# caki35/UNet-Torch

Measured on AMD Instinct MI355X. Metric: images/sec training step, 4-level U-Net 1ch→2cls 512×512, at 1/2/4/8 MI355X, higher is better.
Workload: dtype f16

## Files before the change

unet-torch_amd/csrc/generic_kernels.hip:

```cpp
#include "kernels.h"

template <typename T, bool K8>
__global__ void pack_kn_kernel(const float* __restrict__ src, T* __restrict__ dst, int Tn, int K, int N,
                               long st, long sk, long sn, int flip_t, int Kpad, int Npad) {
    long total = (long)Tn * Kpad * Npad;
    for (long i = (long)blockIdx.x * blockDim.x + threadIdx.x; i < total; i += (long)gridDim.x * blockDim.x) {
        int n, k, t;
        if (K8) {
            int k8 = (int)(i & 7);
            long r = i >> 3;
            n = (int)(r % Npad); r /= Npad;
            int kb = (int)(r % (Kpad / 8));
            t = (int)(r / (Kpad / 8));
            k = kb * 8 + k8;
        } else {
            n = (int)(i % Npad);
            long r = i / Npad;
            k = (int)(r % Kpad);
            t = (int)(r / Kpad);
        }
        float v = 0.f;
        if (k < K && n < N) {
            int ts = flip_t ? (Tn - 1 - t) : t;
            v = src[ts * st + k * sk + n * sn];
// ... 523 lines not shown
            vs[i] = ws[((long)rc * 2 + 0) * C + c];
            vq[i] = ws[((long)rc * 2 + w1) * C + c];
        }
#pragma unroll
        for (int i = 0; i < 8; ++i) asm volatile("" : "+v"(vs[i]), "+v"(vq[i]));
#pragma unroll
        for (int i = 0; i < 8; ++i) { const bool ok = r0 + 256 * i < rows; vs[i] = ok ? vs[i] : 0.f; vq[i] = (ok && out1) ? vq[i] : 0.f; }
#pragma unroll
        for (int i = 0; i < 8; ++i) { s += (double)vs[i]; q += (double)vq[i]; }
    }
    sh[0][tid] = s;
    sh[1][tid] = q;
    __syncthreads();
    for (int o = 128; o > 0; o >>= 1) {
        if (tid < o) { sh[0][tid] += sh[0][tid + o]; sh[1][tid] += sh[1][tid + o]; }
        __syncthreads();
    }
    if (tid == 0) {
        out0[c] = (float)(sh[0][0] * (double)scale);
        if (out1) out1[c] = (float)(sh[1][0] * (double)scale);
    }
}

__global__ __launch_bounds__(256) void reduce_rows2_2d_kernel(const float* __restrict__ ws, int rows, int C,
                                                              float* __restrict__ out0, float* __restrict__ out1,
                                                              float scale, int region) {
    double tot = 0.0;
    if (!red2d_block(ws, rows, C, out1 != nullptr, region, tot)) return;
    const int lane = threadIdx.x & 63, c = blockIdx.x * 32 + (lane & 31);
    if (c < C) {
        if (lane < 32) out0[c] = (float)(tot * (double)scale);
        else if (out1) out1[c] = (float)(tot * (double)scale);
    }
}

__global__ __launch_bounds__(256) void reduce_rows2_wide_kernel(const float* __restrict__ ws, int rows, int C,
                                                                float* __restrict__ out0, float* __restrict__ out1, float scale) {
    const int c = blockIdx.x * 256 + threadIdx.x;
    if (c >= C) return;
    double s = 0.0, q = 0.0;
    for (int r = 0; r < rows; ++r) {
        s += (double)ws[((long)r * 2 + 0) * C + c];
        if (out1) q += (double)ws[((long)r * 2 + 1) * C + c];
    }
    out0[c] = (float)(s * (double)scale);
    if (out1) out1[c] = (float)(q * (double)scale);
}

void umi_launch_reduce_rows2(const float* ws, int rows, int C, float* out0, float* out1, float scale, hipStream_t s) {
    if (rows <= 64 && C >= 4096)
        hipLaunchKernelGGL(reduce_rows2_wide_kernel, dim3((C + 255) / 256), dim3(256), 0, s, ws, rows, C, out0, out1, scale);
    else if (red2d_ok(rows, C))
        hipLaunchKernelGGL(reduce_rows2_2d_kernel, dim3((C + 31) / 32, (rows + RED_RPS - 1) / RED_RPS), dim3(256), 0, s, ws,
                           rows, C, out0, out1, scale, red2d_region());
    else
        hipLaunchKernelGGL(reduce_rows2_kernel, dim3(C), dim3(256), 0, s, ws, rows, C, out0, out1, scale);
}

template <typename T>
__global__ void bn_bwd_apply_kernel(T* __restrict__ da, int ldda, const T* __restrict__ y, int ldy,
                                    const float4* __restrict__ tx, const float* __restrict__ rstd,
                                    const float* __restrict__ sum_dz, const float* __restrict__ sum_dzx, long M, int C) {
    const float invM = 1.f / (float)M;
    long total = M * C;
    for (long i = (long)blockIdx.x * blockDim.x + threadIdx.x; i < total; i += (long)gridDim.x * blockDim.x) {
        int c = (int)(i % C);
        long r = i / C;
        da[r * ldda + c] = umi_bn_dz<T>((float)y[r * ldy + c], (float)da[r * ldda + c], tx[c], rstd[c], sum_dz[c] * invM,
                                        sum_dzx[c] * invM);
    }
}

extern "C" size_t umi_bn_bwd_ws_bytes(long M, int C) {
    const int a = umi_cdiv(M, BNB_RPB), b = umi_cdiv(M, umi_bn_bwd_rpb_f16v(M));
    return (size_t)(a > b ? a : b) * 2 * (size_t)C * sizeof(float);
}

extern "C" int umi_bn_bwd_reduce(const void* da, int ldda, const void* y, int ldy, const void* tx, const float* rstd,
                                 float* sum_dz, float* sum_dzx, long M, int C, int dtype, void* ws, size_t ws_bytes,
                                 umi_stream_t stream) {
    if (!da || !y || !tx || !rstd || M <= 0 || C <= 0) return UMI_ERR_BADARG;
    if (ws_bytes < umi_bn_bwd_ws_bytes(M, C)) return UMI_ERR_WORKSPACE;
    int rows = umi_cdiv(M, BNB_RPB);
    hipStream_t s = (hipStream_t)stream;
    if (dtype == UMI_F16 && umi_bn_bwd_reduce1_f16v(da, ldda, y, ldy, tx, rstd, (float*)ws, M, C, s)) {
        UMI_LAUNCH_CHECK();
        rows = umi_cdiv(M, umi_bn_bwd_rpb_f16v(M));
        umi_launch_reduce_rows2((const float*)ws, rows, C, sum_dz, sum_dzx, 1.f, s);
        UMI_LAUNCH_CHECK();
        return UMI_OK;
    }
    if (dtype == UMI_F32) hipLaunchKernelGGL(bn_bwd_reduce1_kernel<float>, dim3(rows), dim3(256), 0, s, (const float*)da, ldda, (const float*)y, ldy, (const float4*)tx, rstd, (float*)ws, M, C);
    else if (dtype == UMI_F16) hipLaunchKernelGGL(bn_bwd_reduce1_kernel<half_t>, dim3(rows), dim3(256), 0, s, (const half_t*)da, ldda, (const half_t*)y, ldy, (const float4*)tx, rstd, (float*)ws, M, C);
    else return UMI_ERR_BADARG;
    UMI_LAUNCH_CHECK();
    umi_launch_reduce_rows2((const float*)ws, rows, C, sum_dz, sum_dzx, 1.f, s);
    UMI_LAUNCH_CHECK();
    return UMI_OK;
}

extern "C" int umi_bn_bwd_apply(void* da, int ldda, const void* y, int ldy, const void* tx, const float* rstd,
                                const float* sum_dz, const float* sum_dzx, long M, int C, int dtype,
                                umi_stream_t stream) {
    if (!da || !y || !tx || !rstd || M <= 0 || C <= 0) return UMI_ERR_BADARG;
    long total = M * C;
    int grid = (int)((total + 255) / 256);
    if (grid > 16384) grid = 16384;
    hipStream_t s = (hipStream_t)stream;
    if (dtype == UMI_F16 && umi_bn_bwd_apply_f16v(da, ldda, y, ldy, tx, rstd, sum_dz, sum_dzx, M, C, s)) {
        UMI_LAUNCH_CHECK();
        return UMI_OK;
    }
    if (dtype == UMI_F32) hipLaunchKernelGGL(bn_bwd_apply_kernel<float>, dim3(grid), dim3(256), 0, s, (float*)da, ldda, (const float*)y, ldy, (const float4*)tx, rstd, sum_dz, sum_dzx, M, C);
    else if (dtype == UMI_F16) hipLaunchKernelGGL(bn_bwd_apply_kernel<half_t>, dim3(grid), dim3(256), 0, s, (half_t*)da, ldda, (const half_t*)y, ldy, (const float4*)tx, rstd, sum_dz, sum_dzx, M, C);
    else return UMI_ERR_BADARG;
    UMI_LAUNCH_CHECK();
    return UMI_OK;
}

template <typename T>
__global__ __launch_bounds__(256) void colsum1_kernel(const T* __restrict__ x, int ldx, float* __restrict__ ws, long M,
                                                      int C, long rows_per_split, float* __restrict__ out, float scale) {
    __shared__ float red[4][64];
    const int cl = threadIdx.x & 63, rl = threadIdx.x >> 6;
    const int c = blockIdx.x * 64 + cl;
    const long r0 = (long)blockIdx.y * rows_per_split;
    long r1 = r0 + rows_per_split;
    if (r1 > M) r1 = M;
    float s = 0.f;
    if (c < C)
        for (long r = r0 + rl; r < r1; r += 4) s += (float)x[r * ldx + c];
    red[rl][cl] = s;
    __syncthreads();
    if (rl == 0 && c < C) {
        const float t = red[0][cl] + red[1][cl] + red[2][cl] + red[3][cl];
        if (gridDim.y == 1) out[c] = t * scale;
        else ws[((long)blockIdx.y * 2 + 0) * C + c] = t;
    }
}

__global__ void fold_cols_kernel(const float* __restrict__ tmp8, int C, float* __restrict__ out, float scale) {
    const int c = threadIdx.x;
    if (c < C) {
        float s = 0.f;
        for (int k = c; k < 8; k += C) s += tmp8[k];
        out[c] = s * scale;
    }
}

static void colsum_plan(long M, int C, int* splits, long* rps) {
    long ctiles = (C + 63) / 64;
    long want = (1024 + ctiles - 1) / ctiles;
    long maxs = (M + 31) / 32;
    if (want > maxs) want = maxs;
    if (want < 1) want = 1;
    *rps = (M + want - 1) / want;
    *splits = (int)((M + *rps - 1) / *rps);
}

extern "C" size_t umi_colsum_ws_bytes(long M, int C) {
    int splits; long rps;
    colsum_plan(M, C, &splits, &rps);
    const int vrows = umi_colsum_rows_f16v(M, C);
    size_t b = (size_t)(splits > vrows ? splits : vrows) * 2 * (size_t)C * sizeof(float);
    if (C < 8 && 8 % C == 0 && (M * C) % 8 == 0) {
        const size_t b8 = ((size_t)umi_colsum_rows_f16v(M * C / 8, 8) * 2 * 8 + 8) * sizeof(float);
        if (b8 > b) b = b8;
    }
    return b;
}

extern "C" int umi_colsum_group(int n, const void* const* xs, int ldx, float* const* outs, float out_scale, long M, int C,
                                int dtype, void* ws, size_t ws_bytes, umi_stream_t stream) {
    if (n <= 0 || !xs || !outs || M <= 0 || C <= 0 || !ws) return UMI_ERR_BADARG;
    for (int i = 0; i < n; ++i)
        if (!xs[i] || !outs[i]) return UMI_ERR_BADARG;
    if (ws_bytes < (size_t)(n < 16 ? n : 16) * umi_colsum_ws_bytes(M, C)) return UMI_ERR_WORKSPACE;
    if (dtype != UMI_F16 || !umi_colsum_group_f16v(n, xs, ldx, outs, out_scale, (float*)ws, M, C, (hipStream_t)stream))
        return UMI_ERR_UNSUPPORTED;
    UMI_LAUNCH_CHECK();
    return UMI_OK;
}

extern "C" int umi_colsum(const void* x, int ldx, float* out, float out_scale, long M, int C, int dtype, void* ws,
                          size_t ws_bytes, umi_stream_t stream) {
    if (!x || !out || M <= 0 || C <= 0) return UMI_ERR_BADARG;
    if (ws_bytes < umi_colsum_ws_bytes(M, C)) return UMI_ERR_WORKSPACE;
    int splits; long rps;
    colsum_plan(M, C, &splits, &rps);
    hipStream_t s = (hipStream_t)stream;
    if (dtype == UMI_F16 && umi_colsum_f16v(x, ldx, (float*)ws, M, C, s)) {
        UMI_LAUNCH_CHECK();
        umi_launch_reduce_rows2((const float*)ws, umi_colsum_rows_f16v(M, C), C, out, (float*)nullptr, out_scale, s);
        UMI_LAUNCH_CHECK();
        return UMI_OK;
    }
    if (dtype == UMI_F16 && C < 8 && 8 % C == 0 && ldx == C && (M * C) % 8 == 0 &&
        ws_bytes >= ((size_t)umi_colsum_rows_f16v(M * C / 8, 8) * 2 * 8 + 8) * sizeof(float)) {
        const long M8 = M * C / 8;
        float* tmp = (float*)ws + (size_t)umi_colsum_rows_f16v(M8, 8) * 2 * 8;
        if (umi_colsum_f16v(x, 8, (float*)ws, M8, 8, s)) {
            UMI_LAUNCH_CHECK();
            umi_launch_reduce_rows2((const float*)ws, umi_colsum_rows_f16v(M8, 8), 8, tmp, (float*)nullptr, 1.f, s);
            hipLaunchKernelGGL(fold_cols_kernel, dim3(1), dim3(64), 0, s, (const float*)tmp, C, out, out_scale);
            UMI_LAUNCH_CHECK();
            return UMI_OK;
        }
    }
    dim3 grid((C + 63) / 64, splits);
    if (dtype == UMI_F32) hipLaunchKernelGGL(colsum1_kernel<float>, grid, dim3(256), 0, s, (const float*)x, ldx, (float*)ws, M, C, rps, out, out_scale);
    else if (dtype == UMI_F16) hipLaunchKernelGGL(colsum1_kernel<half_t>, grid, dim3(256), 0, s, (const half_t*)x, ldx, (float*)ws, M, C, rps, out, out_scale);
    else return UMI_ERR_BADARG;
    UMI_LAUNCH_CHECK();
    if (splits > 1) {
        umi_launch_reduce_rows2((const float*)ws, splits, C, out, (float*)nullptr, out_scale, s);
        UMI_LAUNCH_CHECK();
    }
    return UMI_OK;
}

template <typename T>
__global__ __launch_bounds__(256) void wgrad_generic_kernel(
    const T* __restrict__ x, int ldx, const float4* __restrict__ txa, const T* __restrict__ dy, int lddy,
    const float4* __restrict__ txb, float* __restrict__ part, int N, int H, int W, int Ci, int Co, int R, int S,
    int stride, int pad, int Ho, int Wo, long chunk, int tiles_co) {
    __shared__ __attribute__((aligned(16))) float As[GBK][64 + 4];
    __shared__ __attribute__((aligned(16))) float Bs[GBK][64 + 4];
    const int tid = threadIdx.x;
    const int txi = tid & 15, tyi = tid >> 4;
    const int tile_ci = blockIdx.x / tiles_co, tile_co = blockIdx.x % tiles_co;
    const int ci0 = tile_ci * 64, co0 = tile_co * 64;
    const int tap = blockIdx.y;
    const int r = tap / S, s = tap - r * S;
    const long P = (long)N * Ho * Wo;
    const long k_begin = (long)blockIdx.z * chunk;
    long k_end = k_begin + chunk;
    if (k_end > P) k_end = P;

    const int lk = tid >> 4;
    const int lc = (tid & 15) * 4;
    float acc[4][4];
#pragma unroll
    for (int i = 0; i < 4; ++i)
#pragma unroll
        for (int j = 0; j < 4; ++j) acc[i][j] = 0.f;

    for (long k0 = k_begin; k0 < k_end; k0 += GBK) {
        long pg = k0 + lk;
        bool pv = pg < k_end;
        int n = 0, ho = 0, wo = 0;
        if (pv) {
            n = (int)(pg / ((long)Ho * Wo));
            int rem = (int)(pg - (long)n * Ho * Wo);
            ho = rem / Wo;
            wo = rem - ho * Wo;
        }
        int hi = ho * stride - pad + r, wi = wo * stride - pad + s;
        bool inb = pv && hi >= 0 && hi < H && wi >= 0 && wi < W;
        const T* xp = x + ((long)((long)n * H + hi) * W + wi) * ldx;
        const T* dp = dy + pg * lddy;
#pragma unroll
        for (int j = 0; j < 4; ++j) {
            int ci = ci0 + lc + j;
            float v = 0.f;
            if (inb && ci < Ci) {
                v = (float)xp[ci];
                if (txa) v = umi_tx(v, txa[ci]);
            }
            As[lk][lc + j] = v;
            int co = co0 + lc + j;
            float g = 0.f;
            if (pv && co < Co) {
                g = (float)dp[co];
                if (txb) g = umi_tx(g, txb[co]);
            }
            Bs[lk][lc + j] = g;
        }
        __syncthreads();
#pragma unroll
        for (int kk = 0; kk < GBK; ++kk) {
            float4 a = *(const float4*)&As[kk][tyi * 4];
            float4 b = *(const float4*)&Bs[kk][txi * 4];
            float av[4] = {a.x, a.y, a.z, a.w};
            float bv[4] = {b.x, b.y, b.z, b.w};
#pragma unroll
            for (int i = 0; i < 4; ++i)
#pragma unroll
                for (int j = 0; j < 4; ++j) acc[i][j] = fmaf(av[i], bv[j], acc[i][j]);
        }
        __syncthreads();
    }
#pragma unroll
    for (int i = 0; i < 4; ++i) {
        int ci = ci0 + tyi * 4 + i;
        if (ci >= Ci) continue;
#pragma unroll
        for (int j = 0; j < 4; ++j) {
            int co = co0 + txi * 4 + j;
            if (co < Co) part[(((long)blockIdx.z * R * S + tap) * Ci + ci) * Co + co] = acc[i][j];
        }
    }
}

__global__ __launch_bounds__(256) void wgrad_reduce_kernel(const float* __restrict__ part, int splits, int RS, int Ci,
                                                           int Co, float* __restrict__ dW, long s_co, long s_ci, long s_t,
                                                           float scale) {
    __shared__ float red[8][33];
    const long total = (long)RS * Ci * Co;
    const int ox = threadIdx.x & 31, sl = threadIdx.x >> 5;
    for (long base = (long)blockIdx.x * 32; base < total; base += (long)gridDim.x * 32) {
        long i = base + ox;
        float s = 0.f;
        if (i < total)
            for (int z = sl; z < splits; z += 8) s += part[(long)z * total + i];
        red[sl][ox] = s;
        __syncthreads();
        if (sl == 0 && i < total) {
            float a = 0.f;
#pragma unroll
            for (int k = 0; k < 8; ++k) a += red[k][ox];
            int co = (int)(i % Co);
            long rr = i / Co;
            int ci = (int)(rr % Ci);
            int t = (int)(rr / Ci);
            dW[co * s_co + ci * s_ci + t * s_t] = a * scale;
        }
        __syncthreads();
    }
}

__global__ __launch_bounds__(256) void wgrad_reduce_v4_kernel(const float* __restrict__ part, int splits, int RS, int Ci,
                                                              int Co, float* __restrict__ dW, long s_co, long s_ci, long s_t,
                                                              float scale) {
    __shared__ float4 red[8][33];
    const long total4 = (long)RS * Ci * Co / 4;
    const int Co4 = Co >> 2;
    const int ox = threadIdx.x & 31, sl = threadIdx.x >> 5;
    for (long base = (long)blockIdx.x * 32; base < total4; base += (long)gridDim.x * 32) {
        const long i = base + ox;
        float4 a = make_float4(0.f, 0.f, 0.f, 0.f), b = a;
        if (i < total4) {
            const float4* p = reinterpret_cast<const float4*>(part) + i;
            int z = sl;
            for (; z + 8 < splits; z += 16) {
                float4 u = p[(long)z * total4], v = p[(long)(z + 8) * total4];
                a.x += u.x; a.y += u.y; a.z += u.z; a.w += u.w;
                b.x += v.x; b.y += v.y; b.z += v.z; b.w += v.w;
            }
            if (z < splits) { float4 u = p[(long)z * total4]; a.x += u.x; a.y += u.y; a.z += u.z; a.w += u.w; }
        }
        red[sl][ox] = make_float4(a.x + b.x, a.y + b.y, a.z + b.z, a.w + b.w);
        __syncthreads();
        if (sl == 0 && i < total4) {
            float4 t4 = red[0][ox];
#pragma unroll
            for (int k = 1; k < 8; ++k) { float4 u = red[k][ox]; t4.x += u.x; t4.y += u.y; t4.z += u.z; t4.w += u.w; }
            const int co = (int)(i % Co4) * 4;
            const long rr = i / Co4;
            const int ci = (int)(rr % Ci), t = (int)(rr / Ci);
            float* o = dW + ci * s_ci + t * s_t;
            o[(co + 0) * s_co] = t4.x * scale;
            o[(co + 1) * s_co] = t4.y * scale;
            o[(co + 2) * s_co] = t4.z * scale;
            o[(co + 3) * s_co] = t4.w * scale;
        }
        __syncthreads();
    }
}

constexpr int WGT_CO = 32, WGT_CI = 8;
__host__ __device__ inline int wg_tmode(const umi_wgrad_pending& d) {
    if (d.Co % WGT_CO || d.Ci % WGT_CI || d.RS > 9 || d.s_t != 1 || (((uintptr_t)d.part) & 15)) return 0;
    if ((long)(d.Co / WGT_CO) * (d.Ci / WGT_CI) < 512) return 0;
    if (d.s_ci == d.RS && d.s_co == (long)d.Ci * d.RS) return 1;
    if (d.s_co == d.RS && d.s_ci == (long)d.Co * d.RS) return 2;
    return 0;
}
__device__ void wg_reduce_tiles(const umi_wgrad_pending& d, int mode, int my_blk, int n_blk) {
    __shared__ float4 redt[8][33];
    __shared__ float tile[WGT_CO * WGT_CI * 9 + 64];
    const int ox = threadIdx.x & 31, sl = threadIdx.x >> 5;
    const int RS = d.RS, ncob = d.Co / WGT_CO, ncib = d.Ci / WGT_CI, rows = WGT_CI * RS;
    const long total4 = (long)RS * d.Ci * d.Co / 4;
    for (int tl = my_blk; tl < ncob * ncib; tl += n_blk) {
        const int cob = tl % ncob, cib = tl / ncob;
        for (int r0 = 0; r0 < rows; r0 += 4) {
            const int row = r0 + (ox >> 3), c4 = ox & 7;
            const int tap = row / WGT_CI, cil = row - tap * WGT_CI;
            float4 a = make_float4(0.f, 0.f, 0.f, 0.f), b = a;
            if (row < rows) {
                const float4* p = reinterpret_cast<const float4*>(d.part) + (((long)tap * d.Ci + cib * WGT_CI + cil) * d.Co + cob * WGT_CO) / 4 + c4;
                int z = sl;
                for (; z + 8 < d.splits; z += 16) {
                    float4 u = p[(long)z * total4], v = p[(long)(z + 8) * total4];
                    a.x += u.x; a.y += u.y; a.z += u.z; a.w += u.w;
                    b.x += v.x; b.y += v.y; b.z += v.z; b.w += v.w;
                }
                if (z < d.splits) { float4 u = p[(long)z * total4]; a.x += u.x; a.y += u.y; a.z += u.z; a.w += u.w; }
                a = make_float4(a.x + b.x, a.y + b.y, a.z + b.z, a.w + b.w);
            }
            redt[sl][ox] = a;
            __syncthreads();
            if (sl == 0 && row < rows) {
                float4 t4 = redt[0][ox];
#pragma unroll
                for (int k = 1; k < 8; ++k) { float4 u = redt[k][ox]; t4.x += u.x; t4.y += u.y; t4.z += u.z; t4.w += u.w; }
                const float v[4] = {t4.x * d.scale, t4.y * d.scale, t4.z * d.scale, t4.w * d.scale};
#pragma unroll
                for (int k = 0; k < 4; ++k) {
                    const int co = c4 * 4 + k;
                    const int idx = mode == 1 ? co * (WGT_CI * RS + 1) + cil * RS + tap : cil * (WGT_CO * RS + 1) + co * RS + tap;
                    tile[idx] = v[k];
                }
            }
            __syncthreads();
        }
        const int inner = mode == 1 ? WGT_CI * RS : WGT_CO * RS, outer = mode == 1 ? WGT_CO : WGT_CI;
        for (int e = threadIdx.x; e < inner * outer; e += 256) {
            const int o = e / inner, r = e - o * inner;
            float* dst = mode == 1 ? d.dW + (long)(cob * WGT_CO + o) * d.s_co + (long)(cib * WGT_CI) * d.s_ci + r
                                   : d.dW + (long)(cib * WGT_CI + o) * d.s_ci + (long)(cob * WGT_CO) * d.s_co + r;
            *dst = tile[o * (inner + 1) + r];
        }
        __syncthreads();
    }
}

struct WgTable { umi_wgrad_pending e[16]; int blk0[17]; };
__global__ __launch_bounds__(256) void wgrad_reduce_group_kernel(WgTable t) {
    __shared__ float4 red[8][33];
    int ent = 0;
#pragma unroll
    for (int i = 1; i < 16; ++i) ent += (int)blockIdx.x >= t.blk0[i];
    const umi_wgrad_pending d = t.e[ent];
    const int my_blk = (int)blockIdx.x - t.blk0[ent], n_blk = t.blk0[ent + 1] - t.blk0[ent];
    if (const int tm = wg_tmode(d)) { wg_reduce_tiles(d, tm, my_blk, n_blk); return; }
    const int ox = threadIdx.x & 31, sl = threadIdx.x >> 5;
    const bool vec = d.Co % 4 == 0 && (((uintptr_t)d.part) & 15) == 0;
    const int W4 = vec ? 4 : 1;
    const long total = (long)d.RS * d.Ci * d.Co / W4;
    const int CoW = d.Co / W4;
    for (long base = (long)my_blk * 32; base < total; base += (long)n_blk * 32) {
        const long i = base + ox;
        float4 a = make_float4(0.f, 0.f, 0.f, 0.f), b = a;
        if (i < total) {
            if (vec) {
                const float4* p = reinterpret_cast<const float4*>(d.part) + i;
                int z = sl;
                for (; z + 8 < d.splits; z += 16) {
                    float4 u = p[(long)z * total], v = p[(long)(z + 8) * total];
                    a.x += u.x; a.y += u.y; a.z += u.z; a.w += u.w;
                    b.x += v.x; b.y += v.y; b.z += v.z; b.w += v.w;
                }
                if (z < d.splits) { float4 u = p[(long)z * total]; a.x += u.x; a.y += u.y; a.z += u.z; a.w += u.w; }
                a = make_float4(a.x + b.x, a.y + b.y, a.z + b.z, a.w + b.w);
            } else {
                for (int z = sl; z < d.splits; z += 8) a.x += d.part[(long)z * total + i];
            }
        }
        red[sl][ox] = a;
        __syncthreads();
        if (sl == 0 && i < total) {
            float4 t4 = red[0][ox];
            if (vec) {
#pragma unroll
                for (int k = 1; k < 8; ++k) { float4 u = red[k][ox]; t4.x += u.x; t4.y += u.y; t4.z += u.z; t4.w += u.w; }
            } else {
                float s0 = 0.f;
#pragma unroll
                for (int k = 0; k < 8; ++k) s0 += red[k][ox].x;
                t4.x = s0;
            }
            const int co = (int)(i % CoW) * W4;
            const long rr = i / CoW;
            const int ci = (int)(rr % d.Ci), tp = (int)(rr / d.Ci);
            float* o = d.dW + ci * d.s_ci + tp * d.s_t;
            o[(co + 0) * d.s_co] = t4.x * d.scale;
            if (vec) {
                o[(co + 1) * d.s_co] = t4.y * d.scale;
                o[(co + 2) * d.s_co] = t4.z * d.scale;
                o[(co + 3) * d.s_co] = t4.w * d.scale;
            }
        }
        __syncthreads();
    }
}

extern "C" int umi_wgrad_reduce_group(int n, const void* items, umi_stream_t stream) {
    if (n <= 0 || !items) return UMI_ERR_BADARG;
    const umi_wgrad_pending* it = (const umi_wgrad_pending*)items;
    for (int i = 0; i < n; ++i)
        if (!it[i].part || !it[i].dW || it[i].splits <= 0 || it[i].RS <= 0 || it[i].Ci <= 0 || it[i].Co <= 0) return UMI_ERR_BADARG;
    for (int g0 = 0; g0 < n; g0 += 16) {
        const int cnt = n - g0 < 16 ? n - g0 : 16;
        WgTable t;
        int total_blk = 0;
        for (int i = 0; i < 16; ++i) {
            t.e[i] = it[g0 + (i < cnt ? i : 0)];
            t.blk0[i] = total_blk;
            if (i >= cnt) continue;
            const bool vec = t.e[i].Co % 4 == 0 && (((uintptr_t)t.e[i].part) & 15) == 0;
            long g = ((long)t.e[i].RS * t.e[i].Ci * t.e[i].Co / (vec ? 4 : 1) + 31) / 32;
            if (wg_tmode(t.e[i])) g = (long)(t.e[i].Co / WGT_CO) * (t.e[i].Ci / WGT_CI);
            total_blk += (int)(g > 4096 ? 4096 : g);
        }
        t.blk0[16] = total_blk;
        hipLaunchKernelGGL(wgrad_reduce_group_kernel, dim3((unsigned)total_blk), dim3(256), 0, (hipStream_t)stream, t);
        UMI_LAUNCH_CHECK();
    }
    return UMI_OK;
}

void umi_launch_wgrad_reduce(int splits, int RS, int Ci, int Co, const WgradOut& o, hipStream_t st) {
    const float* part = (const float*)o.ws;
    float* const dW = o.dW;
    const long s_co = o.s_co, s_ci = o.s_ci, s_t = o.s_t;
    const float scale = o.out_scale;
    if (o.defer) {
        *o.defer = umi_wgrad_pending{part, dW, s_co, s_ci, s_t, scale, splits, RS, Ci, Co};
        return;
    }
    {
        const umi_wgrad_pending one{part, dW, s_co, s_ci, s_t, scale, splits, RS, Ci, Co};
        if (wg_tmode(one)) {
            WgTable t;
            for (int i = 0; i < 16; ++i) { t.e[i] = one; t.blk0[i] = 0; }
            long g = (long)(Co / WGT_CO) * (Ci / WGT_CI);
            if (g > 4096) g = 4096;
            for (int i = 1; i <= 16; ++i) t.blk0[i] = (int)g;
            hipLaunchKernelGGL(wgrad_reduce_group_kernel, dim3((unsigned)g), dim3(256), 0, st, t);
            return;
        }
    }
    if (Co % 4 == 0 && (((uintptr_t)part) & 15) == 0) {
        long g4 = ((long)RS * Ci * Co / 4 + 31) / 32;
        if (g4 > 16384) g4 = 16384;
        hipLaunchKernelGGL(wgrad_reduce_v4_kernel, dim3((unsigned)g4), dim3(256), 0, st, part, splits, RS, Ci, Co, dW, s_co, s_ci, s_t, scale);
        return;
    }
    long total = (long)RS * Ci * Co;
    long g = (total + 31) / 32;
    if (g > 16384) g = 16384;
    hipLaunchKernelGGL(wgrad_reduce_kernel, dim3((unsigned)g), dim3(256), 0, st, part, splits, RS, Ci, Co, dW, s_co, s_ci, s_t, scale);
}


static void wgrad_generic_plan(long P, int Ci, int Co, int RS, int* splits, long* chunk) {
    long tiles = (long)umi_cdiv(Ci, 64) * umi_cdiv(Co, 64) * RS;
    long want = (2048 + tiles - 1) / tiles;
    long maxs = (P + 255) / 256;
    if (want > maxs) want = maxs;
    if (want < 1) want = 1;
    long ch = (P + want - 1) / want;
    ch = (ch + GBK - 1) / GBK * GBK;
    *chunk = ch;
    *splits = (int)((P + ch - 1) / ch);
}

size_t umi_conv_wgrad_generic_ws_bound(const WgradProblem& p) {
    int splits; long chunk;
    wgrad_generic_plan((long)p.N * p.Ho * p.Wo, p.Ci, p.Co, p.R * p.S, &splits, &chunk);
    return (size_t)splits * p.R * p.S * p.Ci * p.Co * sizeof(float);
}

int umi_conv_wgrad_generic(const WgradProblem& p, const void* x, const void* txa, const void* dy, const void* txb,
                           const WgradOut& o, hipStream_t st) {
    const int N = p.N, H = p.H, W = p.W, Ci = p.Ci, Co = p.Co, R = p.R, S = p.S, stride = p.stride, pad = p.pad, Ho = p.Ho, Wo = p.Wo,
              ldx = p.ldx, lddy = p.lddy, dtype = p.dtype;
    void* const ws = o.ws;
    if (o.ws_bytes < umi_conv_wgrad_generic_ws_bound(p)) return UMI_ERR_WORKSPACE;
    int splits; long chunk;
    wgrad_generic_plan((long)N * Ho * Wo, Ci, Co, R * S, &splits, &chunk);
    const int tiles_co = umi_cdiv(Co, 64);
    dim3 grid(umi_cdiv(Ci, 64) * tiles_co, R * S, splits), block(256);
    if (dtype == UMI_F32) hipLaunchKernelGGL(wgrad_generic_kernel<float>, grid, block, 0, st, (const float*)x, ldx, (const float4*)txa, (const float*)dy, lddy, (const float4*)txb, (float*)ws, N, H, W, Ci, Co, R, S, stride, pad, Ho, Wo, chunk, tiles_co);
    else if (dtype == UMI_F16) hipLaunchKernelGGL(wgrad_generic_kernel<half_t>, grid, block, 0, st, (const half_t*)x, ldx, (const float4*)txa, (const half_t*)dy, lddy, (const float4*)txb, (float*)ws, N, H, W, Ci, Co, R, S, stride, pad, Ho, Wo, chunk, tiles_co);
    else return UMI_ERR_BADARG;
    UMI_LAUNCH_CHECK();
    umi_launch_wgrad_reduce(splits, R * S, Ci, Co, o, st);
    UMI_LAUNCH_CHECK();
    return UMI_OK;
}

template <typename T>
__global__ void materialize_nchw_kernel(const T* __restrict__ x, int ldx, const float4* __restrict__ tx,
                                        float* __restrict__ y, int N, int H, int W, int C) {
    long total = (long)N * C * H * W;
    for (long i = (long)blockIdx.x * blockDim.x + threadIdx.x; i < total; i += (long)gridDim.x * blockDim.x) {
        int w = (int)(i % W);
        long r = i / W;
        int h = (int)(r % H);
        r /= H;
        int c = (int)(r % C);
        int n = (int)(r / C);
        float v = (float)x[((long)((long)n * H + h) * W + w) * ldx + c];
        if (tx) v = umi_tx(v, tx[c]);
        y[i] = v;
    }
}

extern "C" int umi_materialize_nchw(const void* x, int ldx, const void* tx, float* y, int N, int H, int W, int C,
                                    int dtype, umi_stream_t stream) {
    if (!x || !y || N <= 0 || H <= 0 || W <= 0 || C <= 0) return UMI_ERR_BADARG;
    long total = (long)N * C * H * W;
    int grid = (int)((total + 255) / 256);
    if (grid > 16384) grid = 16384;
    hipStream_t s = (hipStream_t)stream;
    if (dtype == UMI_F32) hipLaunchKernelGGL(materialize_nchw_kernel<float>, dim3(grid), dim3(256), 0, s, (const float*)x, ldx, (const float4*)tx, y, N, H, W, C);
    else if (dtype == UMI_F16) hipLaunchKernelGGL(materialize_nchw_kernel<half_t>, dim3(grid), dim3(256), 0, s, (const half_t*)x, ldx, (const float4*)tx, y, N, H, W, C);
    else return UMI_ERR_BADARG;
    UMI_LAUNCH_CHECK();
    return UMI_OK;
}
```

Measured before the change: 737.6.

## Rework split-K wgrad reduction with split-count specialized kernels and byte-based grid sizing

Rewrites the weight-gradient split reduction. Small split counts now get a direct per-thread sum with all loads issued up front, and larger counts get multi-element lane reductions whose loads are batched. Grid size is now chosen from the bytes to be reduced against a fixed target grid instead of one block per 32 elements. The aim is more memory-level parallelism and fewer, fuller blocks in a step dominated by small reductions. The costs are more template instantiations, a larger shared-memory footprint per block, and possible under-occupancy for mid-sized layers.

```diff
diff --git a/unet-torch_amd/csrc/generic_kernels.hip b/unet-torch_amd/csrc/generic_kernels.hip
--- a/unet-torch_amd/csrc/generic_kernels.hip
+++ b/unet-torch_amd/csrc/generic_kernels.hip
@@ -849,70 +849,184 @@
     }
 }
 
+__device__ inline void wg_add(float& a, float b) { a += b; }
+__device__ inline void wg_add(float4& a, const float4& b) { a.x += b.x; a.y += b.y; a.z += b.z; a.w += b.w; }
+__device__ inline void wg_keep(float& v) { asm volatile("" : "+v"(v)); }
+__device__ inline void wg_keep(float4& v) { asm volatile("" : "+v"(v.x), "+v"(v.y), "+v"(v.z), "+v"(v.w)); }
+template <typename V> __device__ inline V wg_zero();
+template <> __device__ inline float wg_zero<float>() { return 0.f; }
+template <> __device__ inline float4 wg_zero<float4>() { return make_float4(0.f, 0.f, 0.f, 0.f); }
+
+__host__ __device__ inline int wg_pow2(int splits) { return splits <= 1 ? 1 : splits <= 2 ? 2 : splits <= 4 ? 4 : 8; }
+__host__ __device__ inline int wg_nb(int splits) { return splits <= 8 ? 8 / wg_pow2(splits) : splits <= 16 ? 4 : splits <= 32 ? 2 : 1; }
+__host__ __device__ inline int wg_batch(int splits) { return (splits <= 8 ? 256 : 32) * wg_nb(splits); }
+
+template <typename V, int NB, int L>
+__device__ inline void wg_sum_few(const V* (&p)[NB], long stride, int splits, V (&t)[NB]) {
+    constexpr bool two = sizeof(V) == 16;
+    V x[NB][L];
+#pragma unroll
+    for (int b = 0; b < NB; ++b)
+#pragma unroll
+        for (int l = 0; l < L; ++l) x[b][l] = p[b][(long)(l < splits ? l : splits - 1) * stride];
+#pragma unroll
+    for (int b = 0; b < NB; ++b)
+#pragma unroll
+        for (int l = 0; l < L; ++l) wg_keep(x[b][l]);
+#pragma unroll
+    for (int b = 0; b < NB; ++b) {
+        t[b] = wg_zero<V>();
+#pragma unroll
+        for (int l = 0; l < 8; ++l) {
+            V s = wg_zero<V>();
+            if (l < L) {
+                V xs = s;
+                wg_add(xs, x[b][l < L ? l : 0]);
+                if (l < splits) s = xs;
+            }
+            if (two) wg_add(s, wg_zero<V>());
+            if (two && l == 0) t[b] = s;
+            else wg_add(t[b], s);
+        }
+    }
+}
+
+template <typename V, int NB, int NZ>
+__device__ inline void wg_sum_lane(const V* (&p)[NB], long stride, int sl, int splits, V (&s)[NB]) {
+    constexpr bool two = sizeof(V) == 16;
+    static_assert(NZ % 2 == 0, "a trip starts on a term of chain a");
+    V a[NB], c[NB];
+#pragma unroll
+    for (int b = 0; b < NB; ++b) a[b] = c[b] = wg_zero<V>();
+    for (int z0 = sl; z0 < splits; z0 += 8 * NZ) {
+        V x[NB][NZ];
+#pragma unroll
+        for (int j = 0; j < NZ; ++j) {
+            const int z = z0 + 8 * j;
+            const long off = (long)(z < splits ? z : splits - 1) * stride;
+#pragma unroll
+            for (int b = 0; b < NB; ++b) x[b][j] = p[b][off];
+        }
+#pragma unroll
+        for (int j = 0; j < NZ; ++j)
+#pragma unroll
+            for (int b = 0; b < NB; ++b) wg_keep(x[b][j]);
+#pragma unroll
+        for (int j = 0; j < NZ; ++j) {
+            const bool ok = z0 + 8 * j < splits;
+#pragma unroll
+            for (int b = 0; b < NB; ++b) {
+                V& acc = (two && (j & 1)) ? c[b] : a[b];
+                V n = acc;
+                wg_add(n, x[b][j]);
+                if (ok) acc = n;
+            }
+        }
+    }
+#pragma unroll
+    for (int b = 0; b < NB; ++b) {
+        s[b] = a[b];
+        if (two) wg_add(s[b], c[b]);
+    }
+}
+
+template <typename V>
+__device__ inline V wg_sum_lanes(const V* red, int nslot, int slot) {
+    constexpr bool two = sizeof(V) == 16;
+    V t = two ? red[slot] : wg_zero<V>();
+#pragma unroll
+    for (int k = two ? 1 : 0; k < 8; ++k) wg_add(t, red[k * nslot + slot]);
+    return t;
+}
+
+__device__ inline void wg_store(const umi_wgrad_pending& d, long i, float t) {
+    const int co = (int)(i % d.Co);
+    const long rr = i / d.Co;
+    const int ci = (int)(rr % d.Ci), tp = (int)(rr / d.Ci);
+    d.dW[co * d.s_co + ci * d.s_ci + tp * d.s_t] = t * d.scale;
+}
+__device__ inline void wg_store(const umi_wgrad_pending& d, long i, const float4& t) {
+    const int Co4 = d.Co >> 2;
+    const int co = (int)(i % Co4) * 4;
+    const long rr = i / Co4;
+    const int ci = (int)(rr % d.Ci), tp = (int)(rr / d.Ci);
+    float* o = d.dW + ci * d.s_ci + tp * d.s_t;
+    o[(co + 0) * d.s_co] = t.x * d.scale;
+    o[(co + 1) * d.s_co] = t.y * d.scale;
+    o[(co + 2) * d.s_co] = t.z * d.scale;
+    o[(co + 3) * d.s_co] = t.w * d.scale;
+}
+
+template <typename V, int NB, int L>
+__device__ inline void wg_elems_few(const umi_wgrad_pending& d, int my_blk, int n_blk) {
+    const long total = (long)d.RS * d.Ci * d.Co / (long)(sizeof(V) / 4);
+    const V* part = reinterpret_cast<const V*>(d.part);
+    for (long base = (long)my_blk * (256 * NB); base < total; base += (long)n_blk * (256 * NB)) {
+        const V* p[NB];
+        V t[NB];
+#pragma unroll
+        for (int b = 0; b < NB; ++b) {
+            const long i = base + b * 256 + threadIdx.x;
+            p[b] = part + (i < total ? i : total - 1);
+        }
+        wg_sum_few<V, NB, L>(p, total, d.splits, t);
+#pragma unroll
+        for (int b = 0; b < NB; ++b) {
+            const long i = base + b * 256 + threadIdx.x;
+            if (i < total) wg_store(d, i, t[b]);
+        }
+    }
+}
+template <typename V, int NB, int NZ>
+__device__ inline void wg_elems_many(const umi_wgrad_pending& d, int my_blk, int n_blk, V* red) {
+    const long total = (long)d.RS * d.Ci * d.Co / (long)(sizeof(V) / 4);
+    const V* part = reinterpret_cast<const V*>(d.part);
+    const int ox = threadIdx.x & 31, sl = threadIdx.x >> 5;
+    for (long base = (long)my_blk * (32 * NB); base < total; base += (long)n_blk * (32 * NB)) {
+        const V* p[NB];
+        V s[NB];
+#pragma unroll
+        for (int b = 0; b < NB; ++b) {
+            const long i = base + b * 32 + ox;
+            p[b] = part + (i < total ? i : total - 1);
+        }
+        wg_sum_lane<V, NB, NZ>(p, total, sl, d.splits, s);
+#pragma unroll
+        for (int b = 0; b < NB; ++b) red[sl * (32 * NB) + b * 32 + ox] = s[b];
+        __syncthreads();
+        const long i = base + threadIdx.x;
+        if (threadIdx.x < 32 * NB && i < total) wg_store(d, i, wg_sum_lanes<V>(red, 32 * NB, threadIdx.x));
+        __syncthreads();
+    }
+}
+template <typename V>
+__device__ void wg_reduce_elems(const umi_wgrad_pending& d, int my_blk, int n_blk, V* red) {
+    switch (d.splits <= 8 ? wg_pow2(d.splits) : d.splits <= 16 ? 16 : d.splits <= 32 ? 32 : 64) {
+        case 1: wg_elems_few<V, 8, 1>(d, my_blk, n_blk); break;
+        case 2: wg_elems_few<V, 4, 2>(d, my_blk, n_blk); break;
+        case 4: wg_elems_few<V, 2, 4>(d, my_blk, n_blk); break;
+        case 8: wg_elems_few<V, 1, 8>(d, my_blk, n_blk); break;
+        case 16: wg_elems_many<V, 4, 2>(d, my_blk, n_blk, red); break;
+        case 32: wg_elems_many<V, 2, 4>(d, my_blk, n_blk, red); break;
+        default: wg_elems_many<V, 1, 8>(d, my_blk, n_blk, red); break;
+    }
+}
+
+constexpr int WG_RED = 8 * 32 * 4;
+
 __global__ __launch_bounds__(256) void wgrad_reduce_kernel(const float* __restrict__ part, int splits, int RS, int Ci,
                                                            int Co, float* __restrict__ dW, long s_co, long s_ci, long s_t,
                                                            float scale) {
-    __shared__ float red[8][33];
-    const long total = (long)RS * Ci * Co;
-    const int ox = threadIdx.x & 31, sl = threadIdx.x >> 5;
-    for (long base = (long)blockIdx.x * 32; base < total; base += (long)gridDim.x * 32) {
-        long i = base + ox;
-        float s = 0.f;
-        if (i < total)
-            for (int z = sl; z < splits; z += 8) s += part[(long)z * total + i];
-        red[sl][ox] = s;
-        __syncthreads();
-        if (sl == 0 && i < total) {
-            float a = 0.f;
-#pragma unroll
-            for (int k = 0; k < 8; ++k) a += red[k][ox];
-            int co = (int)(i % Co);
-            long rr = i / Co;
-            int ci = (int)(rr % Ci);
-            int t = (int)(rr / Ci);
-            dW[co * s_co + ci * s_ci + t * s_t] = a * scale;
-        }
-        __syncthreads();
-    }
-}
-
+    __shared__ float red[WG_RED];
+    const umi_wgrad_pending d{part, dW, s_co, s_ci, s_t, scale, splits, RS, Ci, Co};
+    wg_reduce_elems<float>(d, (int)blockIdx.x, (int)gridDim.x, red);
+}
 __global__ __launch_bounds__(256) void wgrad_reduce_v4_kernel(const float* __restrict__ part, int splits, int RS, int Ci,
                                                               int Co, float* __restrict__ dW, long s_co, long s_ci, long s_t,
                                                               float scale) {
-    __shared__ float4 red[8][33];
-    const long total4 = (long)RS * Ci * Co / 4;
-    const int Co4 = Co >> 2;
-    const int ox = threadIdx.x & 31, sl = threadIdx.x >> 5;
-    for (long base = (long)blockIdx.x * 32; base < total4; base += (long)gridDim.x * 32) {
-        const long i = base + ox;
-        float4 a = make_float4(0.f, 0.f, 0.f, 0.f), b = a;
-        if (i < total4) {
-            const float4* p = reinterpret_cast<const float4*>(part) + i;
-            int z = sl;
-            for (; z + 8 < splits; z += 16) {
-                float4 u = p[(long)z * total4], v = p[(long)(z + 8) * total4];
-                a.x += u.x; a.y += u.y; a.z += u.z; a.w += u.w;
-                b.x += v.x; b.y += v.y; b.z += v.z; b.w += v.w;
-            }
-            if (z < splits) { float4 u = p[(long)z * total4]; a.x += u.x; a.y += u.y; a.z += u.z; a.w += u.w; }
-        }
-        red[sl][ox] = make_float4(a.x + b.x, a.y + b.y, a.z + b.z, a.w + b.w);
-        __syncthreads();
-        if (sl == 0 && i < total4) {
-            float4 t4 = red[0][ox];
-#pragma unroll
-            for (int k = 1; k < 8; ++k) { float4 u = red[k][ox]; t4.x += u.x; t4.y += u.y; t4.z += u.z; t4.w += u.w; }
-            const int co = (int)(i % Co4) * 4;
-            const long rr = i / Co4;
-            const int ci = (int)(rr % Ci), t = (int)(rr / Ci);
-            float* o = dW + ci * s_ci + t * s_t;
-            o[(co + 0) * s_co] = t4.x * scale;
-            o[(co + 1) * s_co] = t4.y * scale;
-            o[(co + 2) * s_co] = t4.z * scale;
-            o[(co + 3) * s_co] = t4.w * scale;
-        }
-        __syncthreads();
-    }
+    __shared__ float4 red[WG_RED];
+    const umi_wgrad_pending d{part, dW, s_co, s_ci, s_t, scale, splits, RS, Ci, Co};
+    wg_reduce_elems<float4>(d, (int)blockIdx.x, (int)gridDim.x, red);
 }
 
 constexpr int WGT_CO = 32, WGT_CI = 8;
@@ -923,114 +1037,130 @@
     if (d.s_co == d.RS && d.s_ci == (long)d.Co * d.RS) return 2;
     return 0;
 }
-__device__ void wg_reduce_tiles(const umi_wgrad_pending& d, int mode, int my_blk, int n_blk) {
-    __shared__ float4 redt[8][33];
-    __shared__ float tile[WGT_CO * WGT_CI * 9 + 64];
-    const int ox = threadIdx.x & 31, sl = threadIdx.x >> 5;
-    const int RS = d.RS, ncob = d.Co / WGT_CO, ncib = d.Ci / WGT_CI, rows = WGT_CI * RS;
+__device__ inline const float4* wg_tile_src(const umi_wgrad_pending& d, int cob, int cib, int q) {
+    const int row = q >> 3, c4 = q & 7, tap = row / WGT_CI, cil = row - tap * WGT_CI;
+    return reinterpret_cast<const float4*>(d.part) + (((long)tap * d.Ci + cib * WGT_CI + cil) * d.Co + cob * WGT_CO) / 4 + c4;
+}
+__device__ inline void wg_tile_put(float* tile, int mode, int RS, int q, const float4& t, float scale) {
+    const int row = q >> 3, c4 = q & 7, tap = row / WGT_CI, cil = row - tap * WGT_CI;
+    const float v[4] = {t.x * scale, t.y * scale, t.z * scale, t.w * scale};
+#pragma unroll
+    for (int k = 0; k < 4; ++k) {
+        const int co = c4 * 4 + k;
+        tile[mode == 1 ? co * (WGT_CI * RS + 1) + cil * RS + tap : cil * (WGT_CO * RS + 1) + co * RS + tap] = v[k];
+    }
+}
+__device__ inline void wg_tile_out(const umi_wgrad_pending& d, const float* tile, int mode, int cob, int cib) {
+    const int RS = d.RS, inner = mode == 1 ? WGT_CI * RS : WGT_CO * RS, outer = mode == 1 ? WGT_CO : WGT_CI;
+    for (int e = threadIdx.x; e < inner * outer; e += 256) {
+        const int o = e / inner, r = e - o * inner;
+        float* dst = mode == 1 ? d.dW + (long)(cob * WGT_CO + o) * d.s_co + (long)(cib * WGT_CI) * d.s_ci + r
+                               : d.dW + (long)(cib * WGT_CI + o) * d.s_ci + (long)(cob * WGT_CO) * d.s_co + r;
+        *dst = tile[o * (inner + 1) + r];
+    }
+}
+template <int NB, int L>
+__device__ inline void wg_tiles_few(const umi_wgrad_pending& d, int mode, int my_blk, int n_blk, float* tile) {
+    const int RS = d.RS, ncob = d.Co / WGT_CO, ncib = d.Ci / WGT_CI, npos = WGT_CI * RS * (WGT_CO / 4);
     const long total4 = (long)RS * d.Ci * d.Co / 4;
     for (int tl = my_blk; tl < ncob * ncib; tl += n_blk) {
         const int cob = tl % ncob, cib = tl / ncob;
-        for (int r0 = 0; r0 < rows; r0 += 4) {
-            const int row = r0 + (ox >> 3), c4 = ox & 7;
-            const int tap = row / WGT_CI, cil = row - tap * WGT_CI;
-            float4 a = make_float4(0.f, 0.f, 0.f, 0.f), b = a;
-            if (row < rows) {
-                const float4* p = reinterpret_cast<const float4*>(d.part) + (((long)tap * d.Ci + cib * WGT_CI + cil) * d.Co + cob * WGT_CO) / 4 + c4;
-                int z = sl;
-                for (; z + 8 < d.splits; z += 16) {
-                    float4 u = p[(long)z * total4], v = p[(long)(z + 8) * total4];
-                    a.x += u.x; a.y += u.y; a.z += u.z; a.w += u.w;
-                    b.x += v.x; b.y += v.y; b.z += v.z; b.w += v.w;
-                }
-                if (z < d.splits) { float4 u = p[(long)z * total4]; a.x += u.x; a.y += u.y; a.z += u.z; a.w += u.w; }
-                a = make_float4(a.x + b.x, a.y + b.y, a.z + b.z, a.w + b.w);
-            }
-            redt[sl][ox] = a;
+        for (int q0 = 0; q0 < npos; q0 += 256 * NB) {
+            if (q0 + (int)(threadIdx.x & ~63u) >= npos) continue;
+            const float4* p[NB];
+            float4 t[NB];
+#pragma unroll
+            for (int b = 0; b < NB; ++b) {
+                const int q = q0 + b * 256 + threadIdx.x;
+                p[b] = wg_tile_src(d, cob, cib, q < npos ? q : npos - 1);
+            }
+            wg_sum_few<float4, NB, L>(p, total4, d.splits, t);
+#pragma unroll
+            for (int b = 0; b < NB; ++b) {
+                const int q = q0 + b * 256 + threadIdx.x;
+                if (q < npos) wg_tile_put(tile, mode, RS, q, t[b], d.scale);
+            }
+        }
+        __syncthreads();
+        wg_tile_out(d, tile, mode, cob, cib);
+        __syncthreads();
+    }
+}
+template <int NB, int NZ>
+__device__ inline void wg_tiles_many(const umi_wgrad_pending& d, int mode, int my_blk, int n_blk, float4* red, float* tile) {
+    const int RS = d.RS, ncob = d.Co / WGT_CO, ncib = d.Ci / WGT_CI, npos = WGT_CI * RS * (WGT_CO / 4);
+    const long total4 = (long)RS * d.Ci * d.Co / 4;
+    const int ox = threadIdx.x & 31, sl = threadIdx.x >> 5;
+    for (int tl = my_blk; tl < ncob * ncib; tl += n_blk) {
+        const int cob = tl % ncob, cib = tl / ncob;
+        for (int q0 = 0; q0 < npos; q0 += 32 * NB) {
+            const float4* p[NB];
+            float4 s[NB];
+#pragma unroll
+            for (int b = 0; b < NB; ++b) {
+                const int q = q0 + b * 32 + ox;
+                p[b] = wg_tile_src(d, cob, cib, q < npos ? q : npos - 1);
+            }
+            wg_sum_lane<float4, NB, NZ>(p, total4, sl, d.splits, s);
+#pragma unroll
+            for (int b = 0; b < NB; ++b) red[sl * (32 * NB) + b * 32 + ox] = s[b];
             __syncthreads();
-            if (sl == 0 && row < rows) {
-                float4 t4 = redt[0][ox];
-#pragma unroll
-                for (int k = 1; k < 8; ++k) { float4 u = redt[k][ox]; t4.x += u.x; t4.y += u.y; t4.z += u.z; t4.w += u.w; }
-                const float v[4] = {t4.x * d.scale, t4.y * d.scale, t4.z * d.scale, t4.w * d.scale};
-#pragma unroll
-                for (int k = 0; k < 4; ++k) {
-                    const int co = c4 * 4 + k;
-                    const int idx = mode == 1 ? co * (WGT_CI * RS + 1) + cil * RS + tap : cil * (WGT_CO * RS + 1) + co * RS + tap;
-                    tile[idx] = v[k];
-                }
-            }
+            const int q = q0 + threadIdx.x;
+            if (threadIdx.x < 32 * NB && q < npos) wg_tile_put(tile, mode, RS, q, wg_sum_lanes<float4>(red, 32 * NB, threadIdx.x), d.scale);
             __syncthreads();
         }
-        const int inner = mode == 1 ? WGT_CI * RS : WGT_CO * RS, outer = mode == 1 ? WGT_CO : WGT_CI;
-        for (int e = threadIdx.x; e < inner * outer; e += 256) {
-            const int o = e / inner, r = e - o * inner;
-            float* dst = mode == 1 ? d.dW + (long)(cob * WGT_CO + o) * d.s_co + (long)(cib * WGT_CI) * d.s_ci + r
-                                   : d.dW + (long)(cib * WGT_CI + o) * d.s_ci + (long)(cob * WGT_CO) * d.s_co + r;
-            *dst = tile[o * (inner + 1) + r];
-        }
+        wg_tile_out(d, tile, mode, cob, cib);
         __syncthreads();
+    }
+}
+template <int L>
+__device__ inline void wg_tiles_few_l(const umi_wgrad_pending& d, int mode, int my_blk, int n_blk, float* tile) {
+    const int ppt = (WGT_CI * d.RS * (WGT_CO / 4) + 255) / 256;
+    if (ppt == 1) wg_tiles_few<1, L>(d, mode, my_blk, n_blk, tile);
+    else if (ppt == 2) wg_tiles_few<2, L>(d, mode, my_blk, n_blk, tile);
+    else wg_tiles_few<3, L>(d, mode, my_blk, n_blk, tile);
+}
+__device__ void wg_reduce_tiles(const umi_wgrad_pending& d, int mode, int my_blk, int n_blk, float4* red, float* tile) {
+    switch (d.splits <= 8 ? wg_pow2(d.splits) : d.splits <= 16 ? 16 : d.splits <= 32 ? 32 : 64) {
+        case 1: wg_tiles_few_l<1>(d, mode, my_blk, n_blk, tile); break;
+        case 2: wg_tiles_few_l<2>(d, mode, my_blk, n_blk, tile); break;
+        case 4: wg_tiles_few_l<4>(d, mode, my_blk, n_blk, tile); break;
+        case 8: wg_tiles_few<1, 8>(d, mode, my_blk, n_blk, tile); break;
+        case 16: wg_tiles_many<4, 2>(d, mode, my_blk, n_blk, red, tile); break;
+        case 32: wg_tiles_many<2, 4>(d, mode, my_blk, n_blk, red, tile); break;
+        default: wg_tiles_many<1, 8>(d, mode, my_blk, n_blk, red, tile); break;
     }
 }
 
 struct WgTable { umi_wgrad_pending e[16]; int blk0[17]; };
 __global__ __launch_bounds__(256) void wgrad_reduce_group_kernel(WgTable t) {
-    __shared__ float4 red[8][33];
+    __shared__ float4 red[WG_RED];
+    __shared__ float tile[WGT_CO * WGT_CI * 9 + 64];
     int ent = 0;
 #pragma unroll
     for (int i = 1; i < 16; ++i) ent += (int)blockIdx.x >= t.blk0[i];
     const umi_wgrad_pending d = t.e[ent];
     const int my_blk = (int)blockIdx.x - t.blk0[ent], n_blk = t.blk0[ent + 1] - t.blk0[ent];
-    if (const int tm = wg_tmode(d)) { wg_reduce_tiles(d, tm, my_blk, n_blk); return; }
-    const int ox = threadIdx.x & 31, sl = threadIdx.x >> 5;
+    if (const int tm = wg_tmode(d)) { wg_reduce_tiles(d, tm, my_blk, n_blk, red, tile); return; }
+    if (d.Co % 4 == 0 && (((uintptr_t)d.part) & 15) == 0) wg_reduce_elems<float4>(d, my_blk, n_blk, red);
+    else wg_reduce_elems<float>(d, my_blk, n_blk, reinterpret_cast<float*>(red));
+}
+
+constexpr long WG_GRID = 2560, WG_MIN_BYTES = 32 * 1024;
+static long wg_bytes(const umi_wgrad_pending& d) { return (long)d.splits * d.RS * d.Ci * d.Co * 4; }
+static long wg_units(const umi_wgrad_pending& d) {
+    if (wg_tmode(d)) return (long)(d.Co / WGT_CO) * (d.Ci / WGT_CI);
     const bool vec = d.Co % 4 == 0 && (((uintptr_t)d.part) & 15) == 0;
-    const int W4 = vec ? 4 : 1;
-    const long total = (long)d.RS * d.Ci * d.Co / W4;
-    const int CoW = d.Co / W4;
-    for (long base = (long)my_blk * 32; base < total; base += (long)n_blk * 32) {
-        const long i = base + ox;
-        float4 a = make_float4(0.f, 0.f, 0.f, 0.f), b = a;
-        if (i < total) {
-            if (vec) {
-                const float4* p = reinterpret_cast<const float4*>(d.part) + i;
-                int z = sl;
-                for (; z + 8 < d.splits; z += 16) {
-                    float4 u = p[(long)z * total], v = p[(long)(z + 8) * total];
-                    a.x += u.x; a.y += u.y; a.z += u.z; a.w += u.w;
-                    b.x += v.x; b.y += v.y; b.z += v.z; b.w += v.w;
-                }
-                if (z < d.splits) { float4 u = p[(long)z * total]; a.x += u.x; a.y += u.y; a.z += u.z; a.w += u.w; }
-                a = make_float4(a.x + b.x, a.y + b.y, a.z + b.z, a.w + b.w);
-            } else {
-                for (int z = sl; z < d.splits; z += 8) a.x += d.part[(long)z * total + i];
-            }
-        }
-        red[sl][ox] = a;
-        __syncthreads();
-        if (sl == 0 && i < total) {
-            float4 t4 = red[0][ox];
-            if (vec) {
-#pragma unroll
-                for (int k = 1; k < 8; ++k) { float4 u = red[k][ox]; t4.x += u.x; t4.y += u.y; t4.z += u.z; t4.w += u.w; }
-            } else {
-                float s0 = 0.f;
-#pragma unroll
-                for (int k = 0; k < 8; ++k) s0 += red[k][ox].x;
-                t4.x = s0;
-            }
-            const int co = (int)(i % CoW) * W4;
-            const long rr = i / CoW;
-            const int ci = (int)(rr % d.Ci), tp = (int)(rr / d.Ci);
-            float* o = d.dW + ci * d.s_ci + tp * d.s_t;
-            o[(co + 0) * d.s_co] = t4.x * d.scale;
-            if (vec) {
-                o[(co + 1) * d.s_co] = t4.y * d.scale;
-                o[(co + 2) * d.s_co] = t4.z * d.scale;
-                o[(co + 3) * d.s_co] = t4.w * d.scale;
-            }
-        }
-        __syncthreads();
-    }
+    const long total = (long)d.RS * d.Ci * d.Co / (vec ? 4 : 1), per = wg_batch(d.splits);
+    return (total + per - 1) / per;
+}
+static int wg_blocks(const umi_wgrad_pending& d, long launch_bytes) {
+    long per = (launch_bytes + WG_GRID - 1) / WG_GRID;
+    if (per < WG_MIN_BYTES) per = WG_MIN_BYTES;
+    long g = (wg_bytes(d) + per - 1) / per;
+    const long u = wg_units(d);
+    if (g > u) g = u;
+    return (int)(g < 1 ? 1 : g);
 }
 
 extern "C" int umi_wgrad_reduce_group(int n, const void* items, umi_stream_t stream) {
@@ -1041,15 +1171,14 @@
     for (int g0 = 0; g0 < n; g0 += 16) {
         const int cnt = n - g0 < 16 ? n - g0 : 16;
         WgTable t;
+        long launch_bytes = 0;
+        for (int i = 0; i < cnt; ++i) launch_bytes += wg_bytes(it[g0 + i]);
         int total_blk = 0;
         for (int i = 0; i < 16; ++i) {
             t.e[i] = it[g0 + (i < cnt ? i : 0)];
             t.blk0[i] = total_blk;
             if (i >= cnt) continue;
-            const bool vec = t.e[i].Co % 4 == 0 && (((uintptr_t)t.e[i].part) & 15) == 0;
-            long g = ((long)t.e[i].RS * t.e[i].Ci * t.e[i].Co / (vec ? 4 : 1) + 31) / 32;
-            if (wg_tmode(t.e[i])) g = (long)(t.e[i].Co / WGT_CO) * (t.e[i].Ci / WGT_CI);
-            total_blk += (int)(g > 4096 ? 4096 : g);
+            total_blk += wg_blocks(t.e[i], launch_bytes);
         }
         t.blk0[16] = total_blk;
         hipLaunchKernelGGL(wgrad_reduce_group_kernel, dim3((unsigned)total_blk), dim3(256), 0, (hipStream_t)stream, t);
@@ -1063,31 +1192,23 @@
     float* const dW = o.dW;
     const long s_co = o.s_co, s_ci = o.s_ci, s_t = o.s_t;
     const float scale = o.out_scale;
+    const umi_wgrad_pending one{part, dW, s_co, s_ci, s_t, scale, splits, RS, Ci, Co};
     if (o.defer) {
-        *o.defer = umi_wgrad_pending{part, dW, s_co, s_ci, s_t, scale, splits, RS, Ci, Co};
+        *o.defer = one;
         return;
     }
-    {
-        const umi_wgrad_pending one{part, dW, s_co, s_ci, s_t, scale, splits, RS, Ci, Co};
-        if (wg_tmode(one)) {
-            WgTable t;
-            for (int i = 0; i < 16; ++i) { t.e[i] = one; t.blk0[i] = 0; }
-            long g = (long)(Co / WGT_CO) * (Ci / WGT_CI);
-            if (g > 4096) g = 4096;
-            for (int i = 1; i <= 16; ++i) t.blk0[i] = (int)g;
-            hipLaunchKernelGGL(wgrad_reduce_group_kernel, dim3((unsigned)g), dim3(256), 0, st, t);
-            return;
-        }
+    const int g = wg_blocks(one, wg_bytes(one));
+    if (wg_tmode(one)) {
+        WgTable t;
+        for (int i = 0; i < 16; ++i) { t.e[i] = one; t.blk0[i] = 0; }
+        for (int i = 1; i <= 16; ++i) t.blk0[i] = g;
+        hipLaunchKernelGGL(wgrad_reduce_group_kernel, dim3((unsigned)g), dim3(256), 0, st, t);
+        return;
     }
     if (Co % 4 == 0 && (((uintptr_t)part) & 15) == 0) {
-        long g4 = ((long)RS * Ci * Co / 4 + 31) / 32;
-        if (g4 > 16384) g4 = 16384;
-        hipLaunchKernelGGL(wgrad_reduce_v4_kernel, dim3((unsigned)g4), dim3(256), 0, st, part, splits, RS, Ci, Co, dW, s_co, s_ci, s_t, scale);
+        hipLaunchKernelGGL(wgrad_reduce_v4_kernel, dim3((unsigned)g), dim3(256), 0, st, part, splits, RS, Ci, Co, dW, s_co, s_ci, s_t, scale);
         return;
     }
-    long total = (long)RS * Ci * Co;
-    long g = (total + 31) / 32;
-    if (g > 16384) g = 16384;
     hipLaunchKernelGGL(wgrad_reduce_kernel, dim3((unsigned)g), dim3(256), 0, st, part, splits, RS, Ci, Co, dW, s_co, s_ci, s_t, scale);
 }
 
```

Measured after the change: 739.1, median of 6. About the same (+0.2%).
